# jacketsj/expANN

Measured on AMD Instinct MI355X. Metric: queries/sec at recall@10=1.0 (exact brute force), 1Mxd128 fp32, k=10, higher is better.
Workload: dtype f32; 1 GPU; brute_force_engine L2 N=1000000 d=128 fp32, 10000 batched queries, k=10 (BASELINE configs[1]); n=1000000, d=128, m=10000, k=10, metric=l2, launch=one process, one GPU, devices_visible=1, comm_ranks=0

## Files before the change

### expann_amd/csrc/expann_hip.hip

```cpp
#include "../../include/expann_hip.h"

#include <hip/hip_runtime.h>

#include <algorithm>
#include <cmath>
#include <cstdio>
#include <cstdlib>
#include <cstring>
#include <memory>
#include <mutex>
#include <string>
#include <vector>

#include "host_common.hpp"
#include "scan_f32.hpp"
#include "scan_gemm_bf16.hpp"
#include "scan_gemm_f16.hpp"
#include "scan_gemm_f16x.hpp"
#include "scan_gemm_f16kx.hpp"
#include "scan_direct_f16.hpp"
#include "scan_gemm_i8.hpp"
#include "scan_gemm_i8q.hpp"
#include "scan_gemm_i8w.hpp"
#include "scan_gemm_w8.hpp"
// ... 90 lines not shown
	DevPtr<float> d_bnorm_f16;
	DevPtr<float> d_bns_f16;
	DevPtr<float> d_qnrm;
	DevPtr<float> d_qscale;
	float f16_scale = 0.0f;
	size_t f16_n_pad = 0;
	bool filter_on = false;
	DevPtr<uint32_t> d_filter_bits;
	size_t filter_words = 0;
	DevPtr<uint32_t> d_filter_stat;
	DevPtr<uint32_t> d_filter_list;
	uint32_t filter_list_len = 0, filter_list_stride = 1;
	size_t n_allowed = 0;
	uint32_t filter_residues = 0;
	DevPtr<float> d_bnorm_f16_m;
	DevPtr<float> d_bns_f16_m;
	bool filter_terms_valid = false;
	const float* bnorm_f16() const { return filter_on ? d_bnorm_f16_m.p : d_bnorm_f16.p; }
	const float* bns_f16() const { return filter_on ? d_bns_f16_m.p : d_bns_f16.p; }
	float f16_bnmax = 0.0f;
	DevPtr<void> d_base_i8f;
	DevPtr<int> d_bp_i8f;
	DevPtr<float> d_rw_i8f;
	DevPtr<float> d_i8f_q;
	GrowPtr<void> d_q8f;
	size_t i8f_q_m = 0;
	I8fConsts i8f{};
	int i8f_state = 0;
	DevPtr<float> d_theta;
	DevPtr<int> d_bias_i;
	DevPtr<int> d_qself;
	GrowPtr<void> d_q;
	GrowPtr<uint64_t> d_ids;
	GrowPtr<float> d_dists;
	long opt_query_tile = 0, opt_cand_capacity = 0, opt_sample_ratio = 32;
	long opt_scan_chunks = 0;
	long opt_async = 0;
	bool host_call = false;
	PinPtr<uint32_t> h_flag_ring;
	uint32_t async_pending = 0;
	hipStream_t async_stream = nullptr;
	long opt_xcd_tolerance = 3;
	long opt_latency_mode = 1;
	long opt_debug = 0;
	long opt_sample_frac = 0;
	long opt_sample_run = 1;
	long opt_sample_pass = 1;
	long opt_tail_chunks = 1;
	long opt_persist = 1;
	long opt_ip_rescale = 1;
	long opt_spec_rank = 0;
	long opt_redo_bound = 1;
	long opt_select_overlap = 1;
	long opt_rerank_rounds = 2;
	long opt_rerank_stats = 0;
	hipStream_t side_stream = nullptr;
	hipEvent_t side_ev[2] = {nullptr, nullptr};
	uint64_t stat_redo_queries = 0;
	uint64_t stat_redo_candidates = 0;
	uint64_t stat_rerank_rows = 0;
	uint64_t stat_redo_overflows = 0;
	uint64_t stat_spec_rank = 0;
	long opt_i8_filter = 1;
	long opt_scan_kernel = 0;
	bool profiling = false;
	hipEvent_t ev[kEventPairs][2];
	bool ev_created = false;
	int ev_used = 0;
	expann_profile prof{};
	mutable std::string err;

	int fail(int code, const std::string& msg) const {
		err = msg;
		return code;
	}
};

inline bool f16_rows(const expann_index* h) { return h->dtype == EXPANN_DTYPE_F16; }
inline bool float_rows(const expann_index* h) { return h->dtype == EXPANN_DTYPE_F32 || f16_rows(h); }

namespace expann {
int num_cus(int device) {
	hipDeviceProp_t prop;
	if (hipGetDeviceProperties(&prop, device) != hipSuccess)
		return 256;
	return prop.multiProcessorCount > 0 ? prop.multiProcessorCount : 256;
// ... 616 lines not shown
		sel.wave_done = 2048;
	}
}
using SelectTopkFn = void (*)(SelectParams);
inline SelectTopkFn select_topk_fn(const expann_index* h, const SelectParams& sel) {
	if (sel.tau_f)
		return select_topk_kernel<float, true>;
	return f16_rows(h) ? select_topk_kernel<_Float16> : select_topk_kernel<float>;
}
int launch_select(expann_index* h, SelectParams& sel, size_t m, uint32_t cap, hipStream_t st, uint32_t longest,
                  bool sum_counts) {
	hipStream_t side = nullptr;
	if (h->opt_select_overlap && longest > 512 && cap > 512) {
		if (!h->side_stream) {
			HIP_TRY(h, hipStreamCreateWithFlags(&h->side_stream, hipStreamNonBlocking));
			for (hipEvent_t& e : h->side_ev)
				HIP_TRY(h, hipEventCreateWithFlags(&e, hipEventDisableTiming));
		}
		side = h->side_stream;
		HIP_TRY(h, hipEventRecord(h->side_ev[0], st));
		HIP_TRY(h, hipStreamWaitEvent(side, h->side_ev[0], 0));
	}
	const hipStream_t st2 = side ? side : st;
	if (sum_counts)
		hipLaunchKernelGGL(sum_u32_kernel, dim3(1), dim3(1024), 0, st2, sel.cand_cnt, (uint32_t)m, h->d_total);
	launch_select_wave(sel, m, cap, st, longest, f16_rows(h), side);
	hipLaunchKernelGGL(select_topk_fn(h, sel), dim3((uint32_t)m), dim3(kBlock), sizeof(uint64_t) * cap + 16, st2, sel);
	HIP_TRY(h, hipGetLastError());
	if (side) {
		HIP_TRY(h, hipEventRecord(h->side_ev[1], side));
		HIP_TRY(h, hipStreamWaitEvent(st, h->side_ev[1], 0));
	}
	return EXPANN_OK;
}

int ensure_hit_logs(expann_index* h, uint32_t grid, int waves, size_t m, uint32_t cap, uint32_t n_chunks,
                    uint32_t n_qtiles, uint32_t xcd_map, hipStream_t st, uint4** log, uint32_t** log_cnt,
                    uint32_t* log_cap_out) {
	const uint32_t n_logs = grid * (uint32_t)waves;
	const uint32_t log_cap = std::max<uint32_t>(
	    4096, pow2ceil((uint32_t)std::min<size_t>(4 * ((m * (size_t)cap + n_logs - 1) / n_logs), 1u << 20)));
	const size_t need = (size_t)n_logs * log_cap * 16;
	if (need > h->log_bytes || n_logs > h->log_cnt_n) {
		HIP_TRY(h, hipStreamSynchronize(st));
		h->d_log.reset();
		h->d_log_cnt.reset();
		h->log_bytes = h->log_cnt_n = 0;
		HIP_TRY(h, hipMalloc(&h->d_log, need));
		HIP_TRY(h, hipMalloc(&h->d_log_cnt, sizeof(uint32_t) * n_logs));
		h->log_bytes = need;
// ... 182 lines not shown
constexpr int kStrictReject = -1001;

const GemmI8qVariant* pick_gemm_i8q(const expann_index* h, size_t m, size_t k) {
	if (float_rows(h) || !(h->opt_scan_kernel == 0 || h->opt_scan_kernel == 5))
		return nullptr;
	if (h->opt_scan_kernel == 0 && (m < 96 || h->n < 65536))
		return nullptr;
	if (h->n < 2 * 256 * kF16TB || k > 256)
		return nullptr;
	for (const auto& v : kGemmI8w)
		if (v.d == h->dim && v.mode == h->int_mode)
			return &v;
	for (const auto& v : kGemmI8x)
		if (v.d == h->dim && v.mode == h->int_mode)
			return &v;
	if (any_dim_i8(h->dim, h->int_mode))
		for (const auto& v : kGemmI8KL)
			if (v.mode == h->int_mode)
				return &v;
	return nullptr;
}

constexpr double kI8fClipRms = 5.5;
constexpr double kI8fListRatio = 2.8;
constexpr double kI8fBreakEvenRatio = 3.4;
bool i8f_auto_region(size_t n, size_t m, size_t k) {
	if (k <= 1)
		return n >= 500000 && m >= 2048;
	if (k <= 10)
		return (n >= 1000000 && m >= 4096) || (n >= 2000000 && m >= 2048);
	if (k <= 16)
		return (n >= 2000000 && m >= 2048) || (n >= 1000000 && m >= 10000);
	return false;
}
bool i8f_wanted(const expann_index* h, size_t m, size_t k) {
	if (h->opt_i8_filter == 0 || h->opt_scan_kernel != 0 || h->dtype != EXPANN_DTYPE_F32 ||
	    h->metric != EXPANN_METRIC_L2 || h->dim != 128 || h->u8_exact == 1 || (h->opt_debug & ~16L) != 0 ||
	    h->i8f_state < 0 || k > 256 || h->n < 2 * 256 * kF16TB)
		return false;
	if (h->opt_i8_filter == 2)
		return true;
	return h->i8f_state != 2 && i8f_auto_region(h->n, m, k);
}
uint64_t i8f_cand_limit(const expann_index* h, size_t m, size_t k, uint32_t spec_j = 0) {
	const double rank = spec_j ? (double)spec_j : (double)k;
	return (uint64_t)(kI8fBreakEvenRatio * 1.2 * rank * sample_frac_for(h, k) * (double)m);
}

int ensure_i8f(expann_index* h, hipStream_t st) {
	if (h->i8f_state != 0)
		return EXPANN_OK;
	const size_t nv = h->n * (size_t)h->dim;
	DevBuf tmp;
	HIP_TRY(h, tmp.alloc(16));
	HIP_TRY(h, hipMemsetAsync(tmp.p, 0, 16, st));
	hipLaunchKernelGGL(i8f_stats_kernel, dim3(2048), dim3(kBlock), 0, st, (const float*)h->d_base, nv, tmp.as<double>(),
	                   reinterpret_cast<uint32_t*>(tmp.as<double>() + 1));
	unsigned char hb[16];
	float bnmax = 0.0f;
	HIP_TRY(h, hipMemcpyAsync(hb, tmp.p, 16, hipMemcpyDeviceToHost, st));
	HIP_TRY(h, hipMemcpyAsync(&bnmax, h->d_bnmax + 2, sizeof(float), hipMemcpyDeviceToHost, st));
	HIP_TRY(h, hipStreamSynchronize(st));
	double sumsq;
	float maxabs;
	std::memcpy(&sumsq, hb, 8);
	std::memcpy(&maxabs, hb + 8, 4);
	const double rms = std::sqrt(sumsq / (double)nv);
	const float clip = (float)std::min<double>(maxabs, kI8fClipRms * rms);
	if (!(clip > 0.0f) || !std::isfinite(clip) || !std::isfinite(rms) || !std::isfinite(bnmax)) {
		h->i8f_state = -1;
		return EXPANN_OK;
	}
	h->i8f = i8f_consts(clip / 127.0f, (float)rms, bnmax, h->dim);
	const size_t n_pad = (h->n + kF16TB - 1) / kF16TB * kF16TB;
	HIP_TRY(h, hipMalloc(&h->d_base_i8f, n_pad * (size_t)h->dim));
	HIP_TRY(h, hipMalloc(&h->d_bp_i8f, sizeof(int) * n_pad));
	HIP_TRY(h, hipMalloc(&h->d_rw_i8f, sizeof(float) * h->n));
	HIP_TRY(h, hipMemsetAsync(h->d_base_i8f, 0, n_pad * (size_t)h->dim, st));
	hipLaunchKernelGGL(i8q_bp_kernel, dim3((uint32_t)((n_pad + kBlock - 1) / kBlock)), dim3(kBlock), 0, st,
	                   (const int*)nullptr, (uint32_t)h->n, (uint32_t)n_pad, h->d_bp_i8f.as<int>());
	hipLaunchKernelGGL(i8f_rows_kernel<128>, dim3((uint32_t)((h->n + kRowsPerGroup - 1) / kRowsPerGroup)), dim3(kBlock), 0,
	                   st, (const float*)h->d_base, (uint32_t)h->n, h->i8f, h->d_base_i8f.as<int8_t>(),
	                   h->d_bp_i8f.as<int>(), h->d_rw_i8f.as<float>());
	HIP_TRY(h, hipGetLastError());
	h->i8f_state = 1;
	return EXPANN_OK;
}

int ensure_i8q(expann_index* h, const GemmI8qVariant* gq, hipStream_t st) {
	if (h->d_base_i8q)
		return EXPANN_OK;
	const size_t n_pad = (h->n + gq->tb - 1) / gq->tb * gq->tb;
	const int dq = gq->dq ? gq->dq : h->dim;
	if (h->int_mode != kI8IP && !h->d_bias_i) {
		HIP_TRY(h, hipMalloc(&h->d_bias_i, sizeof(int) * h->n));
		const dim3 grid((uint32_t)((h->n + kRowsPerGroup - 1) / kRowsPerGroup));
		if (gq->self_any)
			hipLaunchKernelGGL(gq->self_any, grid, dim3(kBlock), 0, st, (const void*)h->d_base, (uint32_t)h->n,
			                   h->d_bias_i.as<int>(), (uint32_t)h->dim);
		else
			hipLaunchKernelGGL(gq->self, grid, dim3(kBlock), 0, st, (const void*)h->d_base, (uint32_t)h->n, h->d_bias_i);
	}
	HIP_TRY(h, hipMalloc(&h->d_bp_i8q, sizeof(int) * n_pad));
	hipLaunchKernelGGL(i8q_bp_kernel, dim3((uint32_t)((n_pad + kBlock - 1) / kBlock)), dim3(kBlock), 0,
	                   st, h->int_mode != kI8IP ? h->d_bias_i.as<const int>() : (const int*)nullptr,
	                   (uint32_t)h->n, (uint32_t)n_pad, h->d_bp_i8q);
// ... 367 lines not shown
				sp.g.clk = sclk.as<unsigned long long>();
			}
			hipLaunchKernelGGL(dvs->sample, dim3(wgs), dim3(kBlock), 0, st, sp);
			HIP_TRY(h, hipGetLastError());
			if (sp.g.clk) {
				unsigned long long c[3] = {0, 0, 0};
				HIP_TRY(h, hipStreamSynchronize(st));
				HIP_TRY(h, hipMemcpy(c, sp.g.clk, sizeof(c), hipMemcpyDeviceToHost));
				std::fprintf(stderr, "sample_direct_f16: %u workgroups, stream %.2f us, thresholds %.2f us\n", wgs,
				             (double)(c[1] - c[0]) / 100.0, (double)(c[2] - c[1]) / 100.0);
			}
			*done = true;
			return EXPANN_OK;
		}
	}
	const uint32_t nt = (uint32_t)((h->n + gvf->tb - 1) / gvf->tb);
	const uint32_t run = (uint32_t)h->opt_sample_run;
	uint32_t t_want = std::max<uint32_t>(256, nt / sample_frac_for(h, k));
	const uint32_t live_res = filt ? (uint32_t)__builtin_popcount(h->filter_residues) : 32u;
	if (filt)
		t_want = std::max<uint32_t>(t_want, (uint32_t)std::min<double>(nt, std::ceil(8.0 * (double)k / (gvf->tb * dens))));
	const uint32_t t_sel = t_want / run * run;
	const uint32_t nqt = (uint32_t)((m + gvf->wgq - 1) / gvf->wgq);
	uint32_t chunks = std::max<uint32_t>(1, ((uint32_t)gvf->wg_per_cu * (uint32_t)cus) / nqt);
	chunks = std::max<uint32_t>(chunks, (uint32_t)((8 * k + live_res - 1) / std::max(1u, live_res)));
	chunks = std::min<uint32_t>(chunks, std::min<uint32_t>(64, t_sel / 4));
	if (t_sel * 2 > nt || (size_t)chunks * live_res < need_classes)
		return EXPANN_OK;
	const int ra = ensure_sample(m * (size_t)chunks * 32 * sizeof(float));
	if (ra != EXPANN_OK)
		return ra;
	GemmF16Params fp{};
	fp.base_f16 = h->d_base_f16;
	fp.bnorm = h->bns_f16();
	fp.n_rows = (uint32_t)h->n;
	fp.n_tiles_sel = t_sel;
	fp.tile_stride = nt / t_sel;
	fp.tile_run = run;
	fp.tiles_per_block = (t_sel + chunks - 1) / chunks;
	chunks = (t_sel + fp.tiles_per_block - 1) / fp.tiles_per_block;
	fp.n_qtiles = nqt;
	fp.queries_f16 = h->d_q_split;
	fp.m = (uint32_t)m;
	fp.sample_out = h->d_sample;
	fp.n_chunks = chunks;
	fp.ksteps = (uint32_t)f16_ld(h->dim) / 32;
// ... 389 lines not shown
	if (!gv && !gvi && levels.size() >= 3 && h->opt_sample_pass && !filt) {
		const uint32_t n_groups = (uint32_t)((h->n + kRowsPerGroup - 1) / kRowsPerGroup);
		const uint32_t sel = n_groups / 16;
		uint32_t blocks = std::min<uint32_t>({128u, cap / 16, sel / 8});
		if (blocks * 16 >= 8 * k && blocks >= 16) {
			Level l0;
			l0.n_groups_sel = sel;
			l0.group_stride = 16;
			l0.classmin_blocks = blocks;
			levels.clear();
			levels.push_back(l0);
			levels.push_back(Level{n_groups, 1, 0});
		}
	}
	if (!flags_clean) {
		HIP_TRY(h, hipMemsetAsync(h->d_overflow, 0, sizeof(uint32_t), st));
		HIP_TRY(h, hipMemsetAsync(h->d_total, 0, sizeof(unsigned long long) * 2, st));
	}
	flags_clean = false;
	li_start = 0;
	theta_ready = false;
	i8f_ready = false;
	spec_j = 0;
	if (gvf && h->opt_sample_pass && levels.size() >= 2) {
		const bool spec_form = gvf->hit_log && gvf->scan_redo && (h->opt_debug & ~16L) == 0 && m > 64;
		if (spec_form && !spec_off && !filt && h->opt_spec_rank >= 0 &&
		    (h->opt_spec_rank > 0 || spec_auto_region(h, m, k, i8f && !i8f_off)))
			spec_j = 1;
		const int rs = sampled_pass_f16(h, gvf, m, k, ip, cus, h->d_tau[levels.size() & 1],
		                                h->d_tau_row[levels.size() & 1], st, &theta_ready, i8f && !i8f_off, &i8f_ready,
		                                &spec_j);
		if (rs != EXPANN_OK)
			return rs;
		if (theta_ready)
			li_start = levels.size() - 1;
	}
	h->stat_spec_rank = spec_j ? spec_j : k;
	if (spec_j) {
		redo_slots = spec_redo_slots(m);
		HIP_TRY(h, grow_ws(h, h->d_redo, RedoWs(redo_slots, h->dim, cap).total));
	}
	return EXPANN_OK;
}

int SearchPass::run_level(size_t li) {
	const Level& L = levels[li];
// ... 679 lines not shown
	}
	expann_index* h = new expann_index();
	h->dim = dim;
	h->dtype = dtype;
	h->metric = metric;
	h->device = device;
	h->elem = (dtype == EXPANN_DTYPE_F32) ? 4 : ((dtype == EXPANN_DTYPE_I16 || dtype == EXPANN_DTYPE_F16) ? 2 : 1);
	h->q_elem = (dtype == EXPANN_DTYPE_I8) ? 1 : (dtype == EXPANN_DTYPE_I16 ? 2 : 4);
	h->int_mode = int_mode;
	if (const char* e = std::getenv("EXPANN_TAIL_CHUNKS"))
		h->opt_tail_chunks = std::atol(e);
	if (const char* e = std::getenv("EXPANN_PERSIST"))
		h->opt_persist = std::atol(e);
	if (const char* e = std::getenv("EXPANN_SPEC_RANK"))
		h->opt_spec_rank = std::max(0L, std::atol(e));
	if (const char* e = std::getenv("EXPANN_REDO_BOUND"))
		h->opt_redo_bound = std::atol(e);
	if (const char* e = std::getenv("EXPANN_SELECT_OVERLAP"))
		h->opt_select_overlap = std::atol(e);
	if (const char* e = std::getenv("EXPANN_RERANK_ROUNDS"))
		h->opt_rerank_rounds = std::atol(e) == 1 ? 1 : 2;
	if (const char* e = std::getenv("EXPANN_I8_FILTER"))
		h->opt_i8_filter = std::min(2L, std::max(0L, std::atol(e)));
	if (hipSetDevice(device) != hipSuccess || hipStreamCreate(&h->stream) != hipSuccess) {
		g_create_error = "hipSetDevice/hipStreamCreate failed";
		delete h;
		return EXPANN_ERR_HIP;
	}
	if (hipFuncSetAttribute((const void*)select_topk_kernel<float>, hipFuncAttributeMaxDynamicSharedMemorySize,
	                        (int)(sizeof(uint64_t) * kMaxCap + 16)) != hipSuccess ||
	    hipFuncSetAttribute((const void*)select_topk_kernel<_Float16>, hipFuncAttributeMaxDynamicSharedMemorySize,
	                        (int)(sizeof(uint64_t) * kMaxCap + 16)) != hipSuccess ||
	    hipFuncSetAttribute((const void*)select_topk_kernel<float, true>, hipFuncAttributeMaxDynamicSharedMemorySize,
	                        (int)(sizeof(uint64_t) * kMaxCap + 16)) != hipSuccess) {
		g_create_error = "hipFuncSetAttribute(select_topk_kernel) failed";
		hipStreamDestroy(h->stream);
		delete h;
		return EXPANN_ERR_HIP;
	}
	for (const auto& v : kGemmF16X)
		if (v.d == dim &&
		    (hipFuncSetAttribute((const void*)v.scan, hipFuncAttributeMaxDynamicSharedMemorySize, v.lds) != hipSuccess ||
		     hipFuncSetAttribute((const void*)v.sample, hipFuncAttributeMaxDynamicSharedMemorySize, v.lds) != hipSuccess ||
		     (v.scan_redo &&
		      hipFuncSetAttribute((const void*)v.scan_redo, hipFuncAttributeMaxDynamicSharedMemorySize, v.lds) != hipSuccess))) {
			g_create_error = "hipFuncSetAttribute(scan_gemm_f16x_kernel) failed";
// ... 146 lines not shown
		}
	}
	return EXPANN_OK;
}

int expann_set_base_device(expann_index* h, const void* d_rows, size_t n, uint64_t id_offset) {
	if (!h)
		return EXPANN_ERR_INVALID_ARG;
	if (!d_rows || n == 0)
		return h->fail(EXPANN_ERR_INVALID_ARG, "empty device base");
	if (n >= (1ull << 32) - 32)
		return h->fail(EXPANN_ERR_UNSUPPORTED, "more than 2^32 rows per shard");
	if (h->owns_base && h->d_base)
		hipFree(h->d_base);
	drop_u8_shadow(h);
	h->d_bnorm.reset();
	h->d_bias_i.reset();
	h->d_bnorm_bf.reset();
	h->d_base_split.reset();
	h->d_base_f16.reset();
	h->d_base_i8f.reset();
	h->d_bp_i8f.reset();
	h->d_rw_i8f.reset();
	h->i8f_state = 0;
	if (h->d_base_i8q && h->base_i8q_owned)
		hipFree(h->d_base_i8q);
	h->d_base_i8q = nullptr;
	h->base_i8q_owned = false;
	h->d_bp_i8q.reset();
	h->d_bnorm_f16.reset();
	h->d_bns_f16.reset();
	h->f16_scale = 0.0f;
	h->f16_n_pad = 0;
	drop_row_filter(h);
	h->d_base = const_cast<void*>(d_rows);
	h->owns_base = false;
	h->n = n;
	h->id_offset = id_offset;
	return EXPANN_OK;
}

size_t expann_size(const expann_index* h) { return h ? (h->d_base ? h->n : h->n_staged) : 0; }

int expann_search_device(expann_index* h, const void* d_queries, size_t m, size_t k,
                         uint64_t* d_ids, float* d_dists, void* stream) {
	if (!h)
// ... 308 lines not shown
		float t = 0;
		HIP_TRY(h, hipEventElapsedTime(&t, h->ev[i][0], h->ev[i][1]));
		ms += t;
	}
	h->prof.scan_ms = ms + h->prof_extra_ms;
	*out = h->prof;
	h->ev_used = 0;
	h->prof_extra_ms = 0;
	h->prof = expann_profile{};
	return EXPANN_OK;
}

int expann_get_stat(expann_index* h, const char* name, uint64_t* out) {
	if (!h || !name || !out)
		return EXPANN_ERR_INVALID_ARG;
	if (!std::strcmp(name, "redo_queries"))
		*out = h->stat_redo_queries;
	else if (!std::strcmp(name, "redo_candidates"))
		*out = h->stat_redo_candidates;
	else if (!std::strcmp(name, "redo_overflows"))
		*out = h->stat_redo_overflows;
	else if (!std::strcmp(name, "spec_rank"))
		*out = h->stat_spec_rank;
	else if (!std::strcmp(name, "rerank_rows"))
		*out = h->stat_rerank_rows;
	else if (!std::strcmp(name, "base_bytes"))
		*out = h->d_base ? (uint64_t)h->n * (uint64_t)h->dim * h->elem : 0;
	else if (!std::strcmp(name, "filter_active"))
		*out = h->filter_on ? 1 : 0;
	else if (!std::strcmp(name, "filter_rows"))
		*out = h->filter_on ? h->n_allowed : expann_size(h);
	else
		return h->fail(EXPANN_ERR_INVALID_ARG, std::string("unknown statistic ") + name);
	return EXPANN_OK;
}

uint32_t expann_spec_rank_auto(size_t k, uint32_t sample_frac) {
	return spec_rank_auto(k, sample_frac ? 1.0 / (double)sample_frac : 1.0);
}

namespace {
int set_row_filter(expann_index* h, const uint32_t* bits, size_t n_words, bool on_device, hipStream_t user_st) {
	if (!h)
		return EXPANN_ERR_INVALID_ARG;
	if (!bits)
		return h->fail(EXPANN_ERR_INVALID_ARG, "row filter: NULL bits");
// ... 71 lines not shown
}

int expann_set_option(expann_index* h, const char* name, long value) {
	if (!h || !name)
		return EXPANN_ERR_INVALID_ARG;
	if (!std::strcmp(name, "query_tile"))
		h->opt_query_tile = value;
	else if (!std::strcmp(name, "cand_capacity"))
		h->opt_cand_capacity = value;
	else if (!std::strcmp(name, "debug"))
		h->opt_debug = value;
	else if (!std::strcmp(name, "scan_kernel"))
		h->opt_scan_kernel = value;
	else if (!std::strcmp(name, "f16x") || !std::strcmp(name, "i8x") || !std::strcmp(name, "i8w")) {
		if (value == 0)
			return h->fail(EXPANN_ERR_UNSUPPORTED, std::string(name) + " = 0: the 32 x 32 MFMA forms of rounds 1-2 were removed in round 3");
	}
	else if (!std::strcmp(name, "tail_chunks"))
		h->opt_tail_chunks = value;
	else if (!std::strcmp(name, "persist"))
		h->opt_persist = value;
	else if (!std::strcmp(name, "i8_filter"))
		h->opt_i8_filter = value < 0 ? 0 : (value > 2 ? 2 : value);
	else if (!std::strcmp(name, "spec_rank"))
		h->opt_spec_rank = value < 0 ? 0 : value;
	else if (!std::strcmp(name, "redo_bound"))
		h->opt_redo_bound = value;
	else if (!std::strcmp(name, "select_overlap"))
		h->opt_select_overlap = value;
	else if (!std::strcmp(name, "rerank_rounds"))
		h->opt_rerank_rounds = value == 1 ? 1 : 2;
	else if (!std::strcmp(name, "rerank_stats"))
		h->opt_rerank_stats = value ? 1 : 0;
	else if (!std::strcmp(name, "ip_rescale"))
		h->opt_ip_rescale = value;
	else if (!std::strcmp(name, "sample_pass"))
		h->opt_sample_pass = value;
	else if (!std::strcmp(name, "u8_exact"))
		h->opt_u8_exact = value;
	else if (!std::strcmp(name, "latency_mode"))
		h->opt_latency_mode = value;
	else if (!std::strcmp(name, "async_search"))
		h->opt_async = value;
	else if (!std::strcmp(name, "scan_chunks"))
		h->opt_scan_chunks = value;
	else if (!std::strcmp(name, "xcd_tolerance"))
// ... 14 lines not shown
```

### expann_amd/csrc/scan_gemm_f16.hpp

```cpp
#pragma once
#include "common.hpp"
#include "scan_gemm_bf16.hpp"
#include "scan_gemm_i8f.hpp"
#include "select.hpp"

namespace expann {

typedef _Float16 f16x8 __attribute__((ext_vector_type(8)));

__host__ __device__ inline float gemm_f16_filter_eps(int d) {
	return d <= 256 ? 1.125f * 0.0009765625f
	                : 0.0009765625f + (4.0f + 4.25f * (float)d + 256.0f) * 5.9604644775390625e-08f;
}

__global__ __launch_bounds__(kBlock) void convert_f16_kernel(const float* in, size_t n_values,
                                                             float scale, _Float16* out,
                                                             uint32_t* maxabs_bits) {
	uint32_t b = 0;
	for (size_t i = (size_t)blockIdx.x * kBlock + threadIdx.x; i < n_values;
	     i += (size_t)gridDim.x * kBlock) {
		const float v = in[i];
		out[i] = (_Float16)(v * scale);
		const uint32_t vb = __builtin_bit_cast(uint32_t, v) & 0x7fffffffu;
		b = vb > b ? vb : b;
// ... 389 lines not shown
	uint32_t* cand_cnt;
	const float* qscale;
	int* i8_thp;
	const float* i8_aq;
	const float* i8_wq_in;
	float* i8_wq;
	double i8_inv_2s2;
	uint32_t j;
	float* tau_s;
};
__device__ inline float sample_tau_of(const SampleTauParams& p, float qn, uint32_t ord) {
	float tau = __builtin_inff();
	if (ord != 0) {
		const float g = ordered_to_float(ord);
		if (p.ip)
			tau = 0.5f * (qn * p.eps + p.abs_coef * __builtin_sqrtf(qn)) - g * (0.5f * p.inv_mul);
		else
			tau = qn * (1.0f + p.eps) + p.abs_coef * __builtin_sqrtf(qn) - g * p.inv_mul;
		if (!(tau == tau))
			tau = __builtin_inff();
	}
	return tau;
}
__device__ inline void sample_tau_finish(const SampleTauParams& p, uint32_t qi, uint32_t ord, uint32_t ord_s) {
	const float qn = p.qnrm[qi];
	const float tau_k = sample_tau_of(p, qn, ord);
	const float tau = (p.tau_s && ord_s != ord) ? sample_tau_of(p, qn, ord_s) : tau_k;
	p.tau[qi] = (p.ip && p.qscale) ? tau_k / p.qscale[qi] : tau_k;
	if (p.tau_s)
		p.tau_s[qi] = (p.ip && p.qscale) ? tau / p.qscale[qi] : tau;
	p.tau_row[qi] = 0xFFFFFFFFu;
	p.theta[qi] = p.ip ? (2.0f * tau + qn * p.eps + p.abs_coef * __builtin_sqrtf(qn)) * p.mul
	                   : (tau - (qn * (1.0f - p.eps) - p.abs_coef * __builtin_sqrtf(qn))) * p.mul;
	if (p.i8_thp)
		i8f_thresholds(p.i8_aq[qi], p.i8_wq_in[qi], tau, p.i8_inv_2s2, &p.i8_thp[qi], &p.i8_wq[qi]);
	p.cand_cnt[qi] = 0;
}
__device__ inline void sample_tau_query_wg(const SampleTauParams& p, uint32_t qi, uint32_t* hist, uint32_t* ctl) {
	const uint32_t tid = threadIdx.x;
	const float* v = p.vals + (size_t)qi * p.n_vals;
	uint32_t ord[8];
#pragma unroll
	for (int j = 0; j < 8; ++j) {
		const uint32_t i = j * kBlock + tid;
		ord[j] = i < p.n_vals ? float_to_ordered(v[i]) : 0u;
	}
	uint32_t prefix = 0, mask = 0, krem = p.k;
	for (int pass = 3; pass >= 0; --pass) {
		const int sh = 8 * pass;
		__syncthreads();
// ... 42 lines not shown
	}
	uint32_t ord[PER];
#pragma unroll
	for (int j = 0; j < PER; ++j)
		ord[j] = (uint32_t)(keys[j] >> 32);
	const bool spec = p.tau_s != nullptr && p.j < p.k;
	uint2 kj;
	if (p.k <= 64) {
		kj = wave_kth_largest_sparse_u32<PER>(ord, p.k, scratch, lane, spec ? p.j : 0u);
	} else {
		kj.x = wave_kth_largest_u32<PER>(ord, p.k);
		kj.y = spec ? wave_kth_largest_u32<PER>(ord, p.j) : 0u;
	}
	if (lane == 0)
		sample_tau_finish(p, qi, kj.x, spec ? kj.y : kj.x);
}
template <int PER>
__global__ __launch_bounds__(kBlock) void sample_tau_kernel(SampleTauParams p) {
	__shared__ uint32_t scratch[kBlock / 64][64];
	const uint32_t qi = blockIdx.x * (kBlock / 64) + (threadIdx.x >> 6);
	if (qi >= p.m)
		return;
	sample_tau_query<PER>(p, qi, threadIdx.x & 63, scratch[threadIdx.x >> 6]);
}

struct RedoCompactParams {
	uint32_t* word;
	const uint32_t* list;
	uint32_t n_slots;
	uint32_t row_bytes;
	const void* q16;
	void* rq16;
	const float* qnrm;
	float* r_qnrm;
	const float* tau;
	const float* bound;
	const float* qscale;
	float eps, abs_coef, mul;
	int ip;
	float* r_theta;
	uint32_t* r_cnt;
	const void* q8;
	void* rq8;
	const float* i8_aq;
	const float* i8_wq_in;
	int* r_thp;
// ... 56 lines not shown
```

### expann_amd/csrc/scan_gemm_i8f.hpp

```cpp
#pragma once
#include <cmath>
#include "common.hpp"

namespace expann {

constexpr int kI8fBpMin = -(1 << 29) - (1 << 22);
constexpr int kI8fBpMax = (1 << 29) - (1 << 22);
constexpr int kI8fThpLim = 1 << 29;

struct I8fConsts {
	float s, inv_s;
	double lo;
	double c;
	double inv_lambda;
	double b2;
	double wn;
	double inv_2s2;
	double eta;
};
inline I8fConsts i8f_consts(float s, float rms, float bnmax, int d) {
	I8fConsts k{};
	k.s = s;
	k.inv_s = 1.0f / s;
	const double u = 5.9604644775390625e-08;
	const double eps = ((double)d / 8.0 + 16.0) * u;
	const double lambda = rms > 0.0f ? 1.4 * (double)s / (3.4641016151377544 * (double)rms) : 0.01;
	k.lo = 1.0 - lambda - eps;
	k.c = 1.0 + 1.0 / lambda;
	k.inv_lambda = 1.0 / lambda;
	k.b2 = 2.0 * std::sqrt((double)bnmax * (1.0 + 0x1p-16)) * (1.0 + 0x1p-40);
	k.wn = 2.0 * (lambda + eps);
	k.inv_2s2 = 1.0 / (2.0 * (double)s * (double)s);
	k.eta = ((double)d + 16.0) * 1.401298464324817e-45;
	return k;
}

__device__ inline float f32_step(float f, bool up) {
	if (f == 0.0f)
		return __builtin_bit_cast(float, up ? 1u : 0x80000001u);
	const uint32_t u = __builtin_bit_cast(uint32_t, f);
	return __builtin_bit_cast(float, ((u >> 31) == 0) == up ? u + 1 : u - 1);
}
__device__ inline float f32_down(double x) {
	const float f = (float)x;
	return (double)f > x ? f32_step(f, false) : f;
}
__device__ inline float f32_up(double x) {
	const float f = (float)x;
	return (double)f < x ? f32_step(f, true) : f;
}
__device__ inline int i8f_quant(float x, float inv_s) {
	const float r = __builtin_rintf(x * inv_s);
	return r >= 127.0f ? 127 : (r <= -127.0f ? -127 : (int)r);
}

__global__ __launch_bounds__(kBlock) void i8f_stats_kernel(const float* in, size_t n, double* sumsq, uint32_t* maxabs_bits) {
// ... 8 lines not shown
		b = vb > b ? vb : b;
	}
	for (int off = 32; off > 0; off >>= 1) {
		s += __shfl_xor(s, off);
		const uint32_t o = (uint32_t)__shfl_xor((int)b, off);
		b = o > b ? o : b;
	}
	if ((threadIdx.x & 63) == 0) {
		red[threadIdx.x >> 6] = s;
		redb[threadIdx.x >> 6] = b;
	}
	__syncthreads();
	if (threadIdx.x == 0) {
		for (int w = 1; w < kBlock / 64; ++w) {
			s += red[w];
			b = redb[w] > b ? redb[w] : b;
		}
		atomicAdd(sumsq, s);
		if (b != 0)
			atomicMax(maxabs_bits, b);
	}
}

template <int D>
__global__ __launch_bounds__(kBlock) void i8f_rows_kernel(const float* x, uint32_t n, I8fConsts k, int8_t* out,
                                                          int* bp, float* row_w) {
	static_assert(D % 64 == 0, "whole 4-byte groups per lane");
	constexpr int PER = D / 16;
	const int lane = threadIdx.x & 63, wave = threadIdx.x >> 6;
	const int l = lane & 15, rg = lane >> 4;
	const uint32_t i = blockIdx.x * kRowsPerGroup + wave * kRowsPerWaveStep + rg;
	const uint32_t ii = i < n ? i : n - 1;
	const float* src = x + (size_t)ii * D + l * PER;
	double nn = 0.0, vv = 0.0;
	uint32_t packed[PER / 4];
#pragma unroll
	for (int w = 0; w < PER / 4; ++w) {
		uint32_t pw = 0;
#pragma unroll
		for (int j = 0; j < 4; ++j) {
			const float v = src[4 * w + j];
			const int t = i8f_quant(v, k.inv_s);
			const double e = (double)v - (double)k.s * (double)t;
			nn += (double)v * (double)v;
			vv += e * e;
			pw |= ((uint32_t)t & 0xFFu) << (8 * j);
		}
		packed[w] = pw;
	}
#pragma unroll
	for (int off = 8; off > 0; off >>= 1) {
		nn += __shfl_xor(nn, off);
		vv += __shfl_xor(vv, off);
	}
	if (i >= n)
		return;
	uint32_t* dst = reinterpret_cast<uint32_t*>(out + (size_t)i * D + l * PER);
#pragma unroll
	for (int w = 0; w < PER / 4; ++w)
		dst[w] = packed[w];
	if (l == 0) {
		const double n_lo = nn * (1.0 - 0x1p-40), v_up = vv * (1.0 + 0x1p-40);
		const double xb = (n_lo * k.lo - k.c * v_up) * k.inv_2s2;
		const double xl = xb - (__builtin_fabs(xb) * 0x1p-30 + 0x1p-10);
		if (xl >= (double)kI8fBpMin && xl <= (double)kI8fBpMax) {
			bp[i] = (int)__builtin_floor(xl);
			row_w[i] = f32_up((k.wn * nn * (1.0 + 0x1p-40) + 2.0 * k.c * v_up) * k.inv_2s2 * (1.0 + 0x1p-40));
		} else {
			bp[i] = xl > 0.0 ? kI8fBpMax : kI8fBpMin;
			row_w[i] = __builtin_inff();
		}
	}
}

struct I8fQueryArgs {
	int8_t* q8;
	float* aq;
	float* wq;
	I8fConsts k;
};
template <int D>
__device__ inline void i8f_query_terms(const I8fQueryArgs& a, uint32_t i, uint32_t m, int l, const float* vals) {
	double nn = 0.0, vv = 0.0;
#pragma unroll
	for (int t = 0; t < D / 16; ++t) {
		const float v = vals[t];
		const int q = i8f_quant(v, a.k.inv_s);
		const double e = (double)v - (double)a.k.s * (double)q;
		nn += (double)v * (double)v;
		vv += e * e;
		if (i < m)
			a.q8[(size_t)i * D + l + 16 * t] = (int8_t)q;
	}
#pragma unroll
	for (int off = 8; off > 0; off >>= 1) {
// ... 27 lines not shown
```

Before: 6.768 million queries/s.

## Derive int8-filter sampling thresholds from an int8 centre score with proven bound

Adds an int8 sampling pass. It runs the i8 GEMM sample kernel on the quantized base, using a per-row centre term (rounded norm over 2s^2) and a global max row width. From this it computes both the speculative threshold and a provable k-th threshold, replacing the previous sampling path when the i8 filter is active. It also reruns a trimmed-stats pass to tighten the quantization clip when outliers dominate, and reorders the count-sum launch after select. The intent is a cheaper and tighter threshold estimate, which means fewer candidates. In exchange it adds extra build-time kernels and memory, and the thresholds could be looser if the width bound is large.

```diff
diff --git a/expann_amd/csrc/expann_hip.hip b/expann_amd/csrc/expann_hip.hip
--- a/expann_amd/csrc/expann_hip.hip
+++ b/expann_amd/csrc/expann_hip.hip
@@ -136,6 +136,8 @@
 	DevPtr<void> d_base_i8f;
 	DevPtr<int> d_bp_i8f;
 	DevPtr<float> d_rw_i8f;
+	DevPtr<int> d_cb_i8f;
+	DevPtr<float> d_wbmax_i8f;
 	DevPtr<float> d_i8f_q;
 	GrowPtr<void> d_q8f;
 	size_t i8f_q_m = 0;
@@ -176,6 +178,8 @@
 	uint64_t stat_redo_overflows = 0;
 	uint64_t stat_spec_rank = 0;
 	long opt_i8_filter = 1;
+	long opt_i8_sample = 1;
+	uint64_t stat_i8_sample = 0;
 	long opt_scan_kernel = 0;
 	bool profiling = false;
 	hipEvent_t ev[kEventPairs][2];
@@ -838,10 +842,10 @@
 		HIP_TRY(h, hipStreamWaitEvent(side, h->side_ev[0], 0));
 	}
 	const hipStream_t st2 = side ? side : st;
+	launch_select_wave(sel, m, cap, st, longest, f16_rows(h), side);
+	hipLaunchKernelGGL(select_topk_fn(h, sel), dim3((uint32_t)m), dim3(kBlock), sizeof(uint64_t) * cap + 16, st2, sel);
 	if (sum_counts)
 		hipLaunchKernelGGL(sum_u32_kernel, dim3(1), dim3(1024), 0, st2, sel.cand_cnt, (uint32_t)m, h->d_total);
-	launch_select_wave(sel, m, cap, st, longest, f16_rows(h), side);
-	hipLaunchKernelGGL(select_topk_fn(h, sel), dim3((uint32_t)m), dim3(kBlock), sizeof(uint64_t) * cap + 16, st2, sel);
 	HIP_TRY(h, hipGetLastError());
 	if (side) {
 		HIP_TRY(h, hipEventRecord(h->side_ev[1], side));
@@ -1070,6 +1074,7 @@
 }
 
 constexpr double kI8fClipRms = 5.5;
+constexpr double kI8fTrimEnergy = 1.0 / 16.0;
 constexpr double kI8fListRatio = 2.8;
 constexpr double kI8fBreakEvenRatio = 3.4;
 bool i8f_auto_region(size_t n, size_t m, size_t k) {
@@ -1113,8 +1118,23 @@
 	float maxabs;
 	std::memcpy(&sumsq, hb, 8);
 	std::memcpy(&maxabs, hb + 8, 4);
-	const double rms = std::sqrt(sumsq / (double)nv);
-	const float clip = (float)std::min<double>(maxabs, kI8fClipRms * rms);
+	double rms = std::sqrt(sumsq / (double)nv);
+	float clip = (float)std::min<double>(maxabs, kI8fClipRms * rms);
+	if (maxabs > clip && std::isfinite(clip) && clip > 0.0f) {
+		HIP_TRY(h, hipMemsetAsync(tmp.p, 0, 16, st));
+		hipLaunchKernelGGL(i8f_trimmed_stats_kernel, dim3(2048), dim3(kBlock), 0, st, (const float*)h->d_base, nv, clip,
+		                   tmp.as<double>(), reinterpret_cast<unsigned long long*>(tmp.as<double>() + 1));
+		HIP_TRY(h, hipMemcpyAsync(hb, tmp.p, 16, hipMemcpyDeviceToHost, st));
+		HIP_TRY(h, hipStreamSynchronize(st));
+		double sumsq_in;
+		unsigned long long n_in;
+		std::memcpy(&sumsq_in, hb, 8);
+		std::memcpy(&n_in, hb + 8, 8);
+		if (n_in > 0 && sumsq_in < kI8fTrimEnergy * sumsq) {
+			rms = std::sqrt(sumsq_in / (double)n_in);
+			clip = (float)std::min<double>(maxabs, kI8fClipRms * rms);
+		}
+	}
 	if (!(clip > 0.0f) || !std::isfinite(clip) || !std::isfinite(rms) || !std::isfinite(bnmax)) {
 		h->i8f_state = -1;
 		return EXPANN_OK;
@@ -1124,12 +1144,19 @@
 	HIP_TRY(h, hipMalloc(&h->d_base_i8f, n_pad * (size_t)h->dim));
 	HIP_TRY(h, hipMalloc(&h->d_bp_i8f, sizeof(int) * n_pad));
 	HIP_TRY(h, hipMalloc(&h->d_rw_i8f, sizeof(float) * h->n));
+	HIP_TRY(h, hipMalloc(&h->d_cb_i8f, sizeof(int) * n_pad));
+	HIP_TRY(h, hipMalloc(&h->d_wbmax_i8f, sizeof(float)));
 	HIP_TRY(h, hipMemsetAsync(h->d_base_i8f, 0, n_pad * (size_t)h->dim, st));
-	hipLaunchKernelGGL(i8q_bp_kernel, dim3((uint32_t)((n_pad + kBlock - 1) / kBlock)), dim3(kBlock), 0, st,
-	                   (const int*)nullptr, (uint32_t)h->n, (uint32_t)n_pad, h->d_bp_i8f.as<int>());
+	HIP_TRY(h, hipMemsetAsync(h->d_wbmax_i8f, 0, sizeof(float), st));
+	static_assert(kI8fCbNone == kI8qPadBp, "the padding's row term serves both passes");
+	for (int* terms : {h->d_bp_i8f.as<int>(), h->d_cb_i8f.as<int>()})
+		hipLaunchKernelGGL(i8q_bp_kernel, dim3((uint32_t)((n_pad + kBlock - 1) / kBlock)), dim3(kBlock), 0, st,
+		                   (const int*)nullptr, (uint32_t)h->n, (uint32_t)n_pad, terms);
 	hipLaunchKernelGGL(i8f_rows_kernel<128>, dim3((uint32_t)((h->n + kRowsPerGroup - 1) / kRowsPerGroup)), dim3(kBlock), 0,
 	                   st, (const float*)h->d_base, (uint32_t)h->n, h->i8f, h->d_base_i8f.as<int8_t>(),
-	                   h->d_bp_i8f.as<int>(), h->d_rw_i8f.as<float>());
+	                   h->d_bp_i8f.as<int>(), h->d_rw_i8f.as<float>(), h->d_cb_i8f.as<int>());
+	hipLaunchKernelGGL(i8f_wbmax_kernel, dim3(1024), dim3(kBlock), 0, st, h->d_rw_i8f.as<const float>(), h->d_cb_i8f.as<const int>(),
+	                   (uint32_t)h->n, reinterpret_cast<uint32_t*>(h->d_wbmax_i8f.as<float>()));
 	HIP_TRY(h, hipGetLastError());
 	h->i8f_state = 1;
 	return EXPANN_OK;
@@ -1543,6 +1570,53 @@
 		t_want = std::max<uint32_t>(t_want, (uint32_t)std::min<double>(nt, std::ceil(8.0 * (double)k / (gvf->tb * dens))));
 	const uint32_t t_sel = t_want / run * run;
 	const uint32_t nqt = (uint32_t)((m + gvf->wgq - 1) / gvf->wgq);
+	if (i8f && spec_ok && !filt && gvf->tb == kF16TB && gvf->wgq == kF16TQ && h->opt_i8_sample > 0 &&
+	    (h->opt_i8_sample == 2 || h->opt_spec_rank == 0)) {
+		const uint32_t j = h->opt_spec_rank > 0 ? (uint32_t)std::min<size_t>((size_t)h->opt_spec_rank, k)
+		                                        : spec_rank_auto(k, (double)t_sel / (double)nt);
+		uint32_t ic = std::max<uint32_t>(1, ((uint32_t)kGemmI8F.wg_per_cu_w * (uint32_t)cus) / nqt);
+		ic = std::max<uint32_t>(ic, (uint32_t)((8 * k + 31) / 32));
+		ic = std::min<uint32_t>(ic, std::min<uint32_t>(64, t_sel / 4));
+		if (j < k && t_sel * 2 <= nt && (size_t)ic * 32 >= 8 * k) {
+			GemmI8wParams wsp{};
+			GemmI8qParams& sp = wsp.q;
+			sp.base = h->d_base_i8f;
+			sp.bp = h->d_cb_i8f;
+			sp.n_rows = (uint32_t)h->n;
+			sp.n_tiles_sel = t_sel;
+			sp.tile_stride = nt / t_sel;
+			sp.tile_run = run;
+			sp.tiles_per_block = (t_sel + ic - 1) / ic;
+			ic = (t_sel + sp.tiles_per_block - 1) / sp.tiles_per_block;
+			const int ri = ensure_sample(m * (size_t)ic * 32 * sizeof(int));
+			if (ri != EXPANN_OK)
+				return ri;
+			sp.n_qtiles = nqt;
+			sp.queries = h->d_q8f;
+			sp.m = (uint32_t)m;
+			sp.sample_out = h->d_sample.as<int>();
+			sp.n_chunks = ic;
+			sp.ksteps = (uint32_t)h->dim / 64;
+			hipLaunchKernelGGL(kGemmI8F.sample_w, dim3(ic * nqt), dim3((uint32_t)kGemmI8F.threads_w), kGemmI8F.lds_w, st, wsp);
+			SampleTauI8cParams cp{};
+			cp.t = tp;
+			cp.t.n_vals = ic * 32;
+			cp.t.j = j;
+			cp.t.tau_s = h->d_tau_s;
+			cp.vals = h->d_sample.as<const int>();
+			cp.wb_max = h->d_wbmax_i8f;
+			cp.two_s2 = 2.0 * (double)h->i8f.s * (double)h->i8f.s;
+			hipLaunchKernelGGL(cp.t.n_vals <= 512 ? sample_tau_i8c_kernel<8>
+			                                      : (cp.t.n_vals <= 1024 ? sample_tau_i8c_kernel<16> : sample_tau_i8c_kernel<32>),
+			                   dim3((uint32_t)((m + kBlock / 64 - 1) / (kBlock / 64))), dim3(kBlock), 0, st, cp);
+			HIP_TRY(h, hipGetLastError());
+			*spec_j = j;
+			*done = true;
+			*i8f_done = true;
+			h->stat_i8_sample = 1;
+			return EXPANN_OK;
+		}
+	}
 	uint32_t chunks = std::max<uint32_t>(1, ((uint32_t)gvf->wg_per_cu * (uint32_t)cus) / nqt);
 	chunks = std::max<uint32_t>(chunks, (uint32_t)((8 * k + live_res - 1) / std::max(1u, live_res)));
 	chunks = std::min<uint32_t>(chunks, std::min<uint32_t>(64, t_sel / 4));
@@ -1978,6 +2052,7 @@
 	theta_ready = false;
 	i8f_ready = false;
 	spec_j = 0;
+	h->stat_i8_sample = 0;
 	if (gvf && h->opt_sample_pass && levels.size() >= 2) {
 		const bool spec_form = gvf->hit_log && gvf->scan_redo && (h->opt_debug & ~16L) == 0 && m > 64;
 		if (spec_form && !spec_off && !filt && h->opt_spec_rank >= 0 &&
@@ -2703,6 +2778,8 @@
 		h->opt_rerank_rounds = std::atol(e) == 1 ? 1 : 2;
 	if (const char* e = std::getenv("EXPANN_I8_FILTER"))
 		h->opt_i8_filter = std::min(2L, std::max(0L, std::atol(e)));
+	if (const char* e = std::getenv("EXPANN_I8_SAMPLE"))
+		h->opt_i8_sample = std::min(2L, std::max(0L, std::atol(e)));
 	if (hipSetDevice(device) != hipSuccess || hipStreamCreate(&h->stream) != hipSuccess) {
 		g_create_error = "hipSetDevice/hipStreamCreate failed";
 		delete h;
@@ -2895,6 +2972,8 @@
 	h->d_base_i8f.reset();
 	h->d_bp_i8f.reset();
 	h->d_rw_i8f.reset();
+	h->d_cb_i8f.reset();
+	h->d_wbmax_i8f.reset();
 	h->i8f_state = 0;
 	if (h->d_base_i8q && h->base_i8q_owned)
 		hipFree(h->d_base_i8q);
@@ -3249,6 +3328,8 @@
 		*out = h->stat_redo_overflows;
 	else if (!std::strcmp(name, "spec_rank"))
 		*out = h->stat_spec_rank;
+	else if (!std::strcmp(name, "i8_sample"))
+		*out = h->stat_i8_sample;
 	else if (!std::strcmp(name, "rerank_rows"))
 		*out = h->stat_rerank_rows;
 	else if (!std::strcmp(name, "base_bytes"))
@@ -3366,6 +3447,8 @@
 		h->opt_persist = value;
 	else if (!std::strcmp(name, "i8_filter"))
 		h->opt_i8_filter = value < 0 ? 0 : (value > 2 ? 2 : value);
+	else if (!std::strcmp(name, "i8_sample"))
+		h->opt_i8_sample = value < 0 ? 0 : (value > 2 ? 2 : value);
 	else if (!std::strcmp(name, "spec_rank"))
 		h->opt_spec_rank = value < 0 ? 0 : value;
 	else if (!std::strcmp(name, "redo_bound"))
diff --git a/expann_amd/csrc/scan_gemm_f16.hpp b/expann_amd/csrc/scan_gemm_f16.hpp
--- a/expann_amd/csrc/scan_gemm_f16.hpp
+++ b/expann_amd/csrc/scan_gemm_f16.hpp
@@ -435,10 +435,14 @@
 	}
 	return tau;
 }
+__device__ inline void sample_tau_store(const SampleTauParams& p, uint32_t qi, float qn, float tau_k, float tau);
 __device__ inline void sample_tau_finish(const SampleTauParams& p, uint32_t qi, uint32_t ord, uint32_t ord_s) {
 	const float qn = p.qnrm[qi];
 	const float tau_k = sample_tau_of(p, qn, ord);
 	const float tau = (p.tau_s && ord_s != ord) ? sample_tau_of(p, qn, ord_s) : tau_k;
+	sample_tau_store(p, qi, qn, tau_k, tau);
+}
+__device__ inline void sample_tau_store(const SampleTauParams& p, uint32_t qi, float qn, float tau_k, float tau) {
 	p.tau[qi] = (p.ip && p.qscale) ? tau_k / p.qscale[qi] : tau_k;
 	if (p.tau_s)
 		p.tau_s[qi] = (p.ip && p.qscale) ? tau / p.qscale[qi] : tau;
@@ -527,6 +531,56 @@
 	if (qi >= p.m)
 		return;
 	sample_tau_query<PER>(p, qi, threadIdx.x & 63, scratch[threadIdx.x >> 6]);
+}
+
+struct SampleTauI8cParams {
+	SampleTauParams t;
+	const int* vals;
+	const float* wb_max;
+	double two_s2;
+};
+template <int PER>
+__global__ __launch_bounds__(kBlock) void sample_tau_i8c_kernel(SampleTauI8cParams pc) {
+	__shared__ uint32_t scratch[kBlock / 64][64];
+	const SampleTauParams& p = pc.t;
+	const int lane = threadIdx.x & 63;
+	const uint32_t qi = blockIdx.x * (kBlock / 64) + (threadIdx.x >> 6);
+	if (qi >= p.m)
+		return;
+	const int* v = pc.vals + (size_t)qi * p.n_vals;
+	uint32_t ord[PER];
+#pragma unroll
+	for (int j = 0; j < PER; ++j) {
+		const uint32_t i = j * 64 + lane;
+		const int g = i < p.n_vals ? v[i] : -2147483647 - 1;
+		ord[j] = g < -kI8fCbMax ? 0u : (uint32_t)g ^ 0x80000000u;
+	}
+	uint2 kj;
+	if (p.k <= 64) {
+		kj = wave_kth_largest_sparse_u32<PER>(ord, p.k, scratch[threadIdx.x >> 6], lane, p.j);
+	} else {
+		kj.x = wave_kth_largest_u32<PER>(ord, p.k);
+		kj.y = wave_kth_largest_u32<PER>(ord, p.j);
+	}
+	if (lane == 0) {
+		const float qn = p.qnrm[qi];
+		float tau_k = __builtin_inff(), tau = __builtin_inff();
+		if (kj.x != 0) {
+			const double aq = (double)p.i8_aq[qi], wq = (double)p.i8_wq_in[qi];
+			const double ulp_aq = __builtin_fabs(aq) * 0x1p-23 + 0x1p-149;
+			const double term = pc.two_s2 * ((0.5 + 0x1p-9 + 0.5 * (double)pc.wb_max[0]) - (double)(int)(kj.x ^ 0x80000000u));
+			const double b = aq + ulp_aq + wq + term;
+			tau_k = f32_up(b + (__builtin_fabs(aq) + wq + __builtin_fabs(term)) * 0x1p-40);
+			if (!(tau_k == tau_k))
+				tau_k = __builtin_inff();
+		}
+		if (kj.y != 0) {
+			tau = (float)((double)qn - pc.two_s2 * (double)(int)(kj.y ^ 0x80000000u));
+			if (!(tau == tau))
+				tau = __builtin_inff();
+		}
+		sample_tau_store(p, qi, qn, tau_k, tau);
+	}
 }
 
 struct RedoCompactParams {
diff --git a/expann_amd/csrc/scan_gemm_i8f.hpp b/expann_amd/csrc/scan_gemm_i8f.hpp
--- a/expann_amd/csrc/scan_gemm_i8f.hpp
+++ b/expann_amd/csrc/scan_gemm_i8f.hpp
@@ -7,6 +7,8 @@
 constexpr int kI8fBpMin = -(1 << 29) - (1 << 22);
 constexpr int kI8fBpMax = (1 << 29) - (1 << 22);
 constexpr int kI8fThpLim = 1 << 29;
+constexpr int kI8fCbMax = 1 << 29;
+constexpr int kI8fCbNone = 1 << 30;
 
 struct I8fConsts {
 	float s, inv_s;
@@ -17,6 +19,7 @@
 	double wn;
 	double inv_2s2;
 	double eta;
+	double w_cap;
 };
 inline I8fConsts i8f_consts(float s, float rms, float bnmax, int d) {
 	I8fConsts k{};
@@ -32,6 +35,7 @@
 	k.wn = 2.0 * (lambda + eps);
 	k.inv_2s2 = 1.0 / (2.0 * (double)s * (double)s);
 	k.eta = ((double)d + 16.0) * 1.401298464324817e-45;
+	k.w_cap = 2.0 * (k.wn * (double)d * (double)rms * (double)rms + 2.0 * k.c * (double)d * (double)s * (double)s / 12.0) * k.inv_2s2;
 	return k;
 }
 
@@ -86,9 +90,41 @@
 	}
 }
 
+__global__ __launch_bounds__(kBlock) void i8f_trimmed_stats_kernel(const float* in, size_t n, float limit, double* sumsq,
+                                                                   unsigned long long* count) {
+	__shared__ double red[kBlock / 64];
+	__shared__ unsigned long long redc[kBlock / 64];
+	double s = 0.0;
+	unsigned long long c = 0;
+	for (size_t i = (size_t)blockIdx.x * kBlock + threadIdx.x; i < n; i += (size_t)gridDim.x * kBlock) {
+		const float v = in[i];
+		if (__builtin_fabsf(v) <= limit) {
+			s += (double)v * (double)v;
+			++c;
+		}
+	}
+	for (int off = 32; off > 0; off >>= 1) {
+		s += __shfl_xor(s, off);
+		c += __shfl_xor(c, off);
+	}
+	if ((threadIdx.x & 63) == 0) {
+		red[threadIdx.x >> 6] = s;
+		redc[threadIdx.x >> 6] = c;
+	}
+	__syncthreads();
+	if (threadIdx.x == 0) {
+		for (int w = 1; w < kBlock / 64; ++w) {
+			s += red[w];
+			c += redc[w];
+		}
+		atomicAdd(sumsq, s);
+		atomicAdd(count, c);
+	}
+}
+
 template <int D>
 __global__ __launch_bounds__(kBlock) void i8f_rows_kernel(const float* x, uint32_t n, I8fConsts k, int8_t* out,
-                                                          int* bp, float* row_w) {
+                                                          int* bp, float* row_w, int* cb) {
 	static_assert(D % 64 == 0, "whole 4-byte groups per lane");
 	constexpr int PER = D / 16;
 	const int lane = threadIdx.x & 63, wave = threadIdx.x >> 6;
@@ -130,11 +166,30 @@
 		if (xl >= (double)kI8fBpMin && xl <= (double)kI8fBpMax) {
 			bp[i] = (int)__builtin_floor(xl);
 			row_w[i] = f32_up((k.wn * nn * (1.0 + 0x1p-40) + 2.0 * k.c * v_up) * k.inv_2s2 * (1.0 + 0x1p-40));
+			const double xc = __builtin_rint(nn * k.inv_2s2);
+			cb[i] = (xc <= (double)kI8fCbMax && (double)row_w[i] <= k.w_cap) ? (int)xc : kI8fCbNone;
 		} else {
 			bp[i] = xl > 0.0 ? kI8fBpMax : kI8fBpMin;
 			row_w[i] = __builtin_inff();
-		}
-	}
+			cb[i] = kI8fCbNone;
+		}
+	}
+}
+
+__global__ __launch_bounds__(kBlock) void i8f_wbmax_kernel(const float* row_w, const int* cb, uint32_t n, uint32_t* out_bits) {
+	uint32_t b = 0;
+	for (uint32_t i = blockIdx.x * kBlock + threadIdx.x; i < n; i += gridDim.x * kBlock) {
+		const float w = row_w[i];
+		const uint32_t wb = __builtin_bit_cast(uint32_t, w);
+		if (cb[i] != kI8fCbNone && w >= 0.0f && w < __builtin_inff() && wb > b)
+			b = wb;
+	}
+	for (int off = 32; off > 0; off >>= 1) {
+		const uint32_t o = (uint32_t)__shfl_xor((int)b, off);
+		b = o > b ? o : b;
+	}
+	if ((threadIdx.x & 63) == 0 && b != 0)
+		atomicMax(out_bits, b);
 }
 
 struct I8fQueryArgs {
diff --git a/profiles/i8_sample_c2.py b/profiles/i8_sample_c2.py
--- /dev/null
+++ b/profiles/i8_sample_c2.py
@@ -0,0 +1,32 @@
+import os
+import sys
+
+import numpy as np
+import torch
+
+sys.path.insert(0, os.path.join(os.path.dirname(os.path.abspath(__file__)), ".."))
+from expann_amd import GpuBruteForceEngine
+
+n, d, m, k = 1_000_000, 128, 10_000, 10
+dev = torch.device("cuda", 0)
+g = torch.Generator(device=dev)
+g.manual_seed(1234)
+base = torch.randn(n, d, device=dev, dtype=torch.float32, generator=g).cpu().numpy()
+g.manual_seed(4321)
+queries = torch.randn(m, d, device=dev, dtype=torch.float32, generator=g).cpu().numpy()
+res = {}
+for i8_sample in (1, 0):
+    eng = GpuBruteForceEngine(d, "l2")
+    eng.store_many_vectors(base)
+    eng.build()
+    eng.set_option("i8_sample", i8_sample)
+    eng.set_profiling(True)
+    ids, dists = eng.query_k_batch(queries, k)
+    prof = eng.get_profile()
+    print(f"i8_sample {i8_sample}: {prof['scan_kernel']}, stat i8_sample {eng.get_stat('i8_sample')}, spec_rank "
+          f"{eng.get_stat('spec_rank')}, {prof['candidates'] / m:.1f} candidates per query, redo_queries "
+          f"{eng.get_stat('redo_queries')}, redo_candidates {eng.get_stat('redo_candidates')}, retries {prof['retries']}")
+    res[i8_sample] = (ids, dists)
+    eng.close()
+assert np.array_equal(res[1][0], res[0][0]) and np.array_equal(res[1][1].view(np.uint32), res[0][1].view(np.uint32))
+print("same ids and distance bits")
diff --git a/profiles/i8_sample_model.py b/profiles/i8_sample_model.py
--- /dev/null
+++ b/profiles/i8_sample_model.py
@@ -0,0 +1,91 @@
+#!/usr/bin/env python3
+import numpy as np
+
+N, D, M, K, J = 266_240, 128, 2048, 10, 4
+rng = np.random.RandomState(20261)
+base = rng.standard_normal((N, D)).astype(np.float32)
+queries = rng.standard_normal((M, D)).astype(np.float32)
+
+b64, q64 = base.astype(np.float64), queries.astype(np.float64)
+rms = float(np.sqrt(np.mean(b64 ** 2)))
+s = float(np.float32(min(float(np.abs(base).max()), 5.5 * rms)) / np.float32(127.0))
+lam = 1.4 * s / (np.sqrt(12.0) * rms)
+eps = (D / 8.0 + 16.0) * 2.0 ** -24
+c = 1.0 + 1.0 / lam
+two_s2 = 2.0 * s * s
+bq = np.clip(np.rint(base * np.float32(1.0 / s)), -127, 127)
+qq = np.clip(np.rint(queries * np.float32(1.0 / s)), -127, 127)
+n_b, v_b = (b64 ** 2).sum(1), ((b64 - s * bq) ** 2).sum(1)
+n_q, v_q = (q64 ** 2).sum(1), ((q64 - s * qq) ** 2).sum(1)
+m_q = np.minimum(2.0 * np.sqrt(n_b.max()) * np.sqrt(v_q), v_q / lam)
+a_b, w_b = n_b * (1 - lam - eps) - c * v_b, 2 * (lam + eps) * n_b + 2 * c * v_b
+a_q, w_q = n_q * (1 - lam - eps) - m_q - v_q, 2 * (lam + eps) * n_q + 2 * m_q + 2 * v_q
+cb = np.rint(n_b / two_s2)
+w_cap = 2.0 * (2 * (lam + eps) * D * rms * rms + 2 * c * D * s * s / 12.0)
+seen = w_b <= w_cap
+bqf, qqf = bq.astype(np.float32), qq.astype(np.float32)
+
+
+def blocks(step=16384):
+    for r0 in range(0, N, step):
+        yield r0, min(N, r0 + step)
+
+
+def exact(r0, r1):
+    return n_q[:, None] + n_b[None, r0:r1] - 2.0 * (queries @ base[r0:r1].T).astype(np.float64)
+
+
+def lower(r0, r1):
+    return a_q[:, None] + a_b[None, r0:r1] - two_s2 * (qqf @ bqf[r0:r1].T).astype(np.float64)
+
+
+best = np.full((M, K), np.inf)
+for r0, r1 in blocks():
+    best = np.partition(np.concatenate([best, exact(r0, r1)], 1), K - 1, 1)[:, :K]
+s_k = best.max(1)
+
+nt = N // 64
+t_sel = nt // 16
+rows_of_tile = lambda t: np.arange(64) + (t * (nt // t_sel)) * 64
+
+
+def class_minima(chunks, score):
+    tpb = -(-t_sel // chunks)
+    chunks = -(-t_sel // tpb)
+    out = np.full((M, chunks, 32), np.inf)
+    for t in range(t_sel):
+        r = rows_of_tile(t)
+        v = score(r).reshape(M, 2, 32).min(1)
+        out[:, t // tpb] = np.minimum(out[:, t // tpb], v)
+    return out.reshape(M, -1)
+
+
+sc_exact = lambda r: n_q[:, None] + n_b[None, r] - 2.0 * (queries @ base[r].T).astype(np.float64)
+g_of = lambda r: (qqf @ bqf[r].T).astype(np.float64) - np.where(seen[r], cb[r], 2.0 ** 30)[None, :]
+sc_centre = lambda r: n_q[:, None] - two_s2 * g_of(r)
+sc_upper = lambda r: (a_q + w_q)[:, None] + (a_b + w_b)[None, r] - two_s2 * (qqf @ bqf[r].T).astype(np.float64)
+
+cases = [("exact scores of the sample", 384, sc_exact), ("int8 centre", 384, sc_centre), ("int8 centre", 608, sc_centre),
+         ("int8 upper bound, row by row", 608, sc_upper)]
+taus = []
+for name, classes, fn in cases:
+    taus.append(np.sort(class_minima(classes // 32, fn), 1)[:, J - 1])
+g_k = -np.sort(-(-(class_minima(19, lambda r: -g_of(r)))), 1)[:, K - 1]
+tau_proven = a_q + w_q + two_s2 * (0.5 - g_k) + 0.5 * w_b[seen].max()
+taus.append(tau_proven)
+counts = np.zeros((len(taus), M), np.int64)
+for r0, r1 in blocks():
+    low = lower(r0, r1)
+    for i, t in enumerate(taus):
+        counts[i] += (low <= t[:, None]).sum(1)
+
+lines = [f"N {N} d {D} queries {M} k {K} j {J}: s {s:.5f} lambda {lam:.5f}, mean interval width W_q + W_b "
+         f"{w_q.mean() + w_b.mean():.2f}, sd of (centre - exact) over the sample "
+         f"{np.std(sc_centre(rows_of_tile(7)) - sc_exact(rows_of_tile(7))):.3f}",
+         "thresholds from | classes | queries failing | rows with L <= tau_s per query, mean / max"]
+for i, (name, classes, _) in enumerate(cases):
+    lines.append(f"{name} | {classes} | {100.0 * (s_k > taus[i]).mean():.2f} % | {counts[i].mean():.1f} / {counts[i].max()}")
+lines.append(f"rows left out of the int8 pass (W_b > {w_cap:.2f}): {int((~seen).sum())}; W_b mean {w_b.mean():.2f}, max {w_b.max():.2f}, max of the rows seen {w_b[seen].max():.2f}")
+lines.append(f"proven tau from the k-th class maximum of g (608 classes) + w_b max / 2: valid for "
+             f"{int((tau_proven >= s_k).sum())} of {M} queries; rows with L <= tau per query {counts[-1].mean():.1f} / {counts[-1].max()}")
+print("\n".join(lines))
```

Result: faster. 7.079 million queries/s (median of 6 runs) (+4.6%).
